# griffithlab/regtools

Hardware: AMD Instinct MI355X
Metric: alignments/sec + junctions/sec, junctions extract, 1/2/4/8 MI355X (higher is better)
Workload: dtype u8/u32 integer; 1 GPU; configs[1]: synthetic 50000000-read 101 bp BAM per GPU, ~15% reads with one N-op, junctions extract -s XS; reads_per_gpu=50000000, seed=1, bgzf_members=169426, compressed_bytes_per_gpu=533101619, inflated_bytes_per_gpu=11060000978

## Files before the change

regtools_amd/csrc/kernels.hip:

```cpp
#include "kernels.h"

#include <mutex>
#include <type_traits>

#include "bam_core.h"
#include "inflate_core.h"
#include "inflate_coop.h"
#include "inflate_ring.h"
#include "inflate_wave.h"

namespace rgx {

__device__ __forceinline__ uint32_t lane_id() { return threadIdx.x & 63u; }
__device__ __forceinline__ uint64_t lanemask_lt() { return (1ull << lane_id()) - 1ull; }

__device__ __forceinline__ uint32_t wave_incl_scan(uint32_t v) {
#pragma unroll
    for (int d = 1; d < 64; d <<= 1) {
        uint32_t t = __shfl_up(v, d, 64);
        if ((int)lane_id() >= d) v += t;
    }
    return v;
}

// ... 686 lines not shown
            if (o < w1) r[j] = ld128(arena + o);
        }
#pragma unroll
        for (int j = 0; j < kChunks; ++j) {
            const uint64_t o = w0 + (uint64_t)j * 1024 + (uint64_t)lane * 16;
            if (o < w1) *(u32x4 *)(s_buf + (o - w0)) = r[j];
        }
    }
    __syncthreads();
    const uint32_t *s_w = (const uint32_t *)s_buf;
    auto lds32 = [&](uint32_t off) -> uint32_t {
        if constexpr (STAGED) return __builtin_amdgcn_alignbyte(s_w[(off >> 2) + 1], s_w[off >> 2], off & 3u);
        else return ld32(arena + w0 + off);
    };
    if (lane * 8 < cnt) {
        uint64_t o = a + seg_cp[(size_t)s * kSegCpSlots + lane];
        const uint32_t k_end = min(cnt, lane * 8 + 8);
        for (uint32_t k = lane * 8; k < k_end; ++k) {
            const uint32_t ro = (uint32_t)(o - w0);
            s_off[k] = ro;
            o += 4 + (uint64_t)((STAGED && o + 4 <= w1) ? lds32(ro) : ld32(arena + o));
        }
    }
    __syncthreads();
    const uint32_t base = seg_base[s];
    DecodeTally t;
    for (uint32_t k = lane; k < cnt; k += 64) {
        const uint32_t ro = s_off[k];
        const uint64_t o = w0 + ro;
        RecHead h;
        {
            const uint32_t sh = ro & 3u, wi = ro >> 2;
            uint32_t x[8];
            if constexpr (STAGED) {
                uint32_t d[9];
#pragma unroll
                for (int q = 0; q < 9; ++q) d[q] = s_w[wi + q];
#pragma unroll
                for (int q = 0; q < 8; ++q) x[q] = __builtin_amdgcn_alignbyte(d[q + 1], d[q], sh);
            } else {
                (void)sh; (void)wi;
#pragma unroll
                for (int q = 0; q < 8; ++q) x[q] = ld32(arena + o + 4 * q);
            }
            rec_head_words(x, h);
        }
        const uint64_t rec_end = o + 4 + (uint64_t)(uint32_t)h.block_len;
        const bool in_win = STAGED && rec_end <= w1;
        const uint32_t cig_ro = ro + 36 + h.l_qname;
        const uint8_t *g_data = arena + o + 36;
        auto cigar_at = [&](uint32_t q) -> uint32_t { return in_win ? lds32(cig_ro + 4 * q) : ld32(g_data + h.l_qname + 4 * (size_t)q); };
        auto tag_strand = [&](uint8_t t0, uint8_t t1, bool *unknown) -> char {
            const int64_t l_data = (int64_t)h.block_len - 32;
            if (in_win) { const uint8_t *body = s_buf + ro + 36; return strand_from_tag(body + h.aux_off, body + l_data, t0, t1, unknown); }
            return strand_from_tag(g_data + h.aux_off, g_data + l_data, t0, t1, unknown);
        };
        decode_record(h, base + k, o, cfg, soa, t, cigar_at, tag_strand);
    }
    const uint32_t n_iter = wave_incl_scan(t.n_iter), n_long = wave_incl_scan(t.n_long);
    if (lane == 63) { seg_iter[s] = n_iter; seg_long[s] = n_long; }
    if (cfg.stop_out) stop_reduce(cfg.stop_out, t.first_stop, t.last_in);
}

__global__ __launch_bounds__(64) void k_decode_sparse(const uint8_t *__restrict__ arena, uint32_t n_seg, const uint64_t *__restrict__ seg_start,
                                                      const uint32_t *__restrict__ seg_base, const uint32_t *__restrict__ seg_cnt, ExtractCfg cfg, ReadSoA soa,
                                                      uint32_t *seg_iter, uint32_t *seg_long, uint32_t s_begin) {
    const uint32_t s = s_begin + blockIdx.x * 64 + threadIdx.x;
    DecodeTally t;
    if (s < n_seg) {
        const uint32_t cnt = seg_cnt[s];
        uint64_t o = cnt ? seg_start[s] : 0;
        const uint32_t base = cnt ? seg_base[s] : 0;
        for (uint32_t k = 0; k < cnt; ++k) {
            RecHead h;
            rec_head(arena + o, h);
            const uint8_t *g_data = arena + o + 36;
            auto cigar_at = [&](uint32_t q) -> uint32_t { return ld32(g_data + h.l_qname + 4 * (size_t)q); };
            auto tag_strand = [&](uint8_t t0, uint8_t t1, bool *unknown) -> char {
                return strand_from_tag(g_data + h.aux_off, g_data + ((int64_t)h.block_len - 32), t0, t1, unknown);
            };
            decode_record(h, base + k, o, cfg, soa, t, cigar_at, tag_strand);
            o += 4 + (uint64_t)(uint32_t)h.block_len;
        }
        seg_iter[s] = t.n_iter; seg_long[s] = t.n_long;
    }
    if (cfg.stop_out) stop_reduce(cfg.stop_out, t.first_stop, t.last_in);
}

__global__ __launch_bounds__(64) void k_long_fill(uint32_t n_seg, const uint32_t *__restrict__ seg_base, const uint32_t *__restrict__ seg_cnt,
                                                  const uint32_t *__restrict__ seg_long_base, ExtractCfg cfg, ReadSoA soa, uint32_t *long_list) {
    const uint32_t s = blockIdx.x, lane = threadIdx.x;
    const uint32_t cnt = seg_cnt[s], base = seg_base[s];
    uint32_t out = seg_long_base[s];
    for (uint32_t k0 = 0; k0 < cnt; k0 += 64) {
        const uint32_t k = k0 + lane;
        bool is_long = false;
        if (k < cnt) is_long = soa.n_ev[base + k] != 0 && (soa.flag_nc[base + k] & 0xffff) > cfg.long_threshold;
        const uint64_t m = __ballot(is_long);
        if (is_long) long_list[out + (uint32_t)__popcll(m & lanemask_lt())] = base + k;
        out += (uint32_t)__popcll(m);
    }
}

const DecodeKnobs &decode_knobs() {
    static const DecodeKnobs k = [] {
        DecodeKnobs v;
        if (const char *e = getenv("REGTOOLS_AMD_DECODE")) {
            v.wave_form = !strncmp(e, "wave", 4);
            if (const char *c = strchr(e, ',')) v.seg_bytes = atoi(c + 1);
        }
        return v;
    }();
    return k;
}
void launch_decode_seg(const uint8_t *arena, SegGeom g, uint32_t n_seg, const uint64_t *seg_start, const uint32_t *seg_base,
                       const uint32_t *seg_cnt, ExtractCfg cfg, ReadSoA soa, uint32_t *seg_iter, uint32_t *seg_long, const uint16_t *seg_cp, bool staged, hipStream_t stream,
                       uint32_t s_begin) {
    if (n_seg <= s_begin) return;
    const uint32_t n = n_seg - s_begin;
    if (staged && g.seg_bytes == kSegBytes) hipLaunchKernelGGL(k_decode_seg<true>, dim3(n), dim3(64), kSegBytes + kSegTail + 48, stream, arena, g, n_seg, seg_start, seg_base, seg_cnt, cfg, soa, seg_iter, seg_long, seg_cp, s_begin);
    else {
        static const bool wave_form = decode_knobs().wave_form;
        if (wave_form && g.seg_bytes == kSegBytes) hipLaunchKernelGGL(k_decode_seg<false>, dim3(n), dim3(64), 0, stream, arena, g, n_seg, seg_start, seg_base, seg_cnt, cfg, soa, seg_iter, seg_long, seg_cp, s_begin);
        else hipLaunchKernelGGL(k_decode_sparse, dim3((n + 63) / 64), dim3(64), 0, stream, arena, n_seg, seg_start, seg_base, seg_cnt, cfg, soa, seg_iter, seg_long, s_begin);
    }
}
__global__ void k_collect_odd_aux(const uint8_t *__restrict__ arena, ReadSoA soa, uint32_t n_rec, uint32_t cap, uint32_t *count, int32_t *out) {
    const uint32_t i = blockIdx.x * blockDim.x + threadIdx.x;
    if (i >= n_rec || !(soa.strand[i] & 0x80u)) return;
    const uint32_t fnc = soa.flag_nc[i];
    const int32_t pos = soa.pos[i];
    const uint32_t k = atomicAdd(count, 1u);
    if (k < cap) { out[3 * (size_t)k] = soa.tid[i]; out[3 * (size_t)k + 1] = pos; out[3 * (size_t)k + 2] = rec_endpos(arena + soa.cig_off[i], fnc & 0xffffu, fnc >> 16, pos); }
}
void launch_collect_odd_aux(const uint8_t *arena, ReadSoA soa, uint32_t n_rec, uint32_t cap, uint32_t *count, int32_t *out, hipStream_t stream) {
    if (n_rec) hipLaunchKernelGGL(k_collect_odd_aux, dim3((n_rec + 255) / 256), dim3(256), 0, stream, arena, soa, n_rec, cap, count, out);
}
void launch_long_fill(uint32_t n_seg, const uint32_t *seg_base, const uint32_t *seg_cnt, const uint32_t *seg_long_base, ExtractCfg cfg, ReadSoA soa,
                      uint32_t *long_list, hipStream_t stream) {
    if (n_seg) hipLaunchKernelGGL(k_long_fill, dim3(n_seg), dim3(64), 0, stream, n_seg, seg_base, seg_cnt, seg_long_base, cfg, soa, long_list);
}


__device__ __forceinline__ void put_event(const EventSoA &ev, uint32_t slot, int32_t tid, uint32_t start, uint32_t end, uint32_t ts,
                                          uint32_t te, char strand, uint32_t rpos, uint32_t rend, uint32_t read) {
    if (ev.read) ev.read[slot] = read;
    ev.tid[slot] = (uint32_t)tid; ev.start[slot] = start;
    ev.ilen_cls[slot] = (end - start) << 2 | strand_class(strand);
    ev.ts[slot] = ts; ev.te[slot] = te; ev.strand[slot] = (uint8_t)strand;
    if (ev.rpos) { ev.rpos[slot] = rpos; ev.rend[slot] = rend; }
}

__global__ void k_emit_short(const uint8_t *__restrict__ arena, uint32_t n_rec, ExtractCfg cfg, ReadSoA soa,
                             const uint32_t *__restrict__ ev_base, EventSoA ev, uint32_t row_begin, const uint32_t *__restrict__ part_totals, uint32_t n_parts, uint32_t slot_cap) {
    uint32_t i = row_begin + blockIdx.x * blockDim.x + threadIdx.x;
    if (i >= n_rec) return;
    uint32_t nev = soa.n_ev[i];
    if (!nev) return;
    uint32_t fnc = soa.flag_nc[i], n_cigar = fnc & 0xffff;
    if (n_cigar > cfg.long_threshold) return;
    const uint8_t *cig = arena + soa.cig_off[i];
    int32_t tid = soa.tid[i];
    char strand = (char)soa.strand[i];
    uint32_t slot = ev_base[i];
    for (uint32_t k = 0; k < n_parts; ++k) slot += part_totals[k];
    const int32_t pos = soa.pos[i];
    const uint32_t rend = ev.rpos ? (uint32_t)rec_endpos(cig, n_cigar, fnc >> 16, pos) : 0u;
    char carried = 0;
    cigar_walk(pos, cig, n_cigar, [&](uint32_t s, uint32_t e, uint32_t ts, uint32_t te) {
        char st = strand;
        if (cfg.fa_data) {
            const FaContig fc = cfg.fa_tab[tid];
            if (!fc.present) { cfg.fa_missing[0] = 1u + (uint32_t)tid; }
            else { const char m = strand_from_motif(cfg.fa_data, fc, s, e, carried); if (m != '?') st = m; }
            carried = st;
        }
        if (intron_ok(s, e, cfg.min_intron, cfg.max_intron)) { if (slot < slot_cap) put_event(ev, slot, tid, s, e, ts, te, st, (uint32_t)pos, rend, i); ++slot; }
    });
}

__global__ __launch_bounds__(256) void k_emit_long(const uint8_t *__restrict__ arena, const uint32_t *__restrict__ long_list,
                                                   uint32_t n_long, ExtractCfg cfg, ReadSoA soa,
                                                   const uint32_t *__restrict__ ev_base, EventSoA ev) {
    __shared__ uint32_t s_ops[4][64];
    __shared__ uint32_t s_R[4][65];
    const uint32_t wave = threadIdx.x >> 6, lane = lane_id();
    const uint32_t stride = gridDim.x * 4;
    uint32_t w = blockIdx.x * 4 + wave;
    if (w >= n_long) return;
    uint32_t nx_i = long_list[w];
    uint32_t nn_i = w + stride < n_long ? long_list[w + stride] : 0u;
    uint32_t nx_fnc = soa.flag_nc[nx_i], nx_slot = ev_base[nx_i];
    uint64_t nx_cig = soa.cig_off[nx_i];
    int32_t nx_tid = soa.tid[nx_i], nx_pos = soa.pos[nx_i];
    uint8_t nx_strand = soa.strand[nx_i];
    for (; w < n_long; w += stride) {
        const uint32_t i = nx_i, fnc = nx_fnc;
        const uint32_t n_cigar = fnc & 0xffff;
        const uint8_t *cig = arena + nx_cig;
        const int32_t tid = nx_tid;
        const char strand = (char)nx_strand;
        uint32_t slot = nx_slot;
        const uint32_t rpos = (uint32_t)nx_pos;
        const uint32_t c_first = lane < n_cigar ? ld32(cig + 4 * (size_t)lane) : 0x5u ;
        if (w + stride < n_long) {
            nx_i = nn_i;
            nx_fnc = soa.flag_nc[nx_i]; nx_slot = ev_base[nx_i]; nx_cig = soa.cig_off[nx_i]; nx_tid = soa.tid[nx_i]; nx_pos = soa.pos[nx_i]; nx_strand = soa.strand[nx_i];
            if (w + 2 * stride < n_long) nn_i = long_list[w + 2 * stride];
        }
        uint32_t rend = 0;
        if (ev.rpos) {
            uint32_t span = 0;
            for (uint32_t t0 = lane; t0 < n_cigar; t0 += 64) span += cig_ref_len(ld32(cig + 4 * (size_t)t0));
            span = __shfl(wave_incl_scan(span), 63, 64);
            rend = ((fnc >> 16) & 4u) ? rpos + 1 : rpos + span;
        }
        uint32_t refpos = rpos;
        uint32_t ts_carry = refpos;
        bool pend = false; uint32_t p_start = 0, p_end = 0, p_ts = 0; char p_strand = strand;
        char carried = 0;
        for (uint32_t t0 = 0; t0 < n_cigar; t0 += 64) {
            const uint32_t k = t0 + lane;
            const uint32_t c = t0 == 0 ? c_first : k < n_cigar ? ld32(cig + 4 * (size_t)k) : 0x5u ;
            s_ops[wave][lane] = c;
            const uint32_t adv = cig_advances_junction_state(c) ? (c >> 4) : 0u;
            const uint32_t incl = wave_incl_scan(adv);
            const uint32_t R_before = refpos + incl - adv, R_after = refpos + incl;
            s_R[wave][lane] = R_before;
            if (lane == 63) s_R[wave][64] = R_after;
            const bool brk = k < n_cigar && cig_is_breaker(c);
            const bool isN = k < n_cigar && cig_is_N(c);
            const uint64_t B = __ballot(brk);
            __builtin_amdgcn_wave_barrier();
            if (pend && B) {
                const uint32_t nb = (uint32_t)__ffsll((unsigned long long)B) - 1;
                const uint32_t te = s_R[wave][nb];
                if (lane == 0 && intron_ok(p_start, p_end, cfg.min_intron, cfg.max_intron)) put_event(ev, slot, tid, p_start, p_end, p_ts, te, p_strand, rpos, rend, i);
                if (intron_ok(p_start, p_end, cfg.min_intron, cfg.max_intron)) ++slot;
                pend = false;
            }
            const uint64_t below = B & lanemask_lt();
            const uint64_t above = lane == 63 ? 0ull : (B >> (lane + 1)) << (lane + 1);
            const uint32_t ts = below ? s_R[wave][(63 - (uint32_t)__clzll((long long)below)) + 1] : ts_carry;
            const bool closed = above != 0;
            const uint32_t te = closed ? s_R[wave][(uint32_t)__ffsll((unsigned long long)above) - 1] : 0u;
            const bool ok = isN && intron_ok(R_before, R_after, cfg.min_intron, cfg.max_intron);
            char my_strand = strand;
            if (cfg.fa_data) {
                const FaContig fc = cfg.fa_tab[tid];
                char sA = strand, sB = strand;
                if (isN) {
                    if (!fc.present) cfg.fa_missing[0] = 1u + (uint32_t)tid;
                    else {
                        const char mA = strand_from_motif(cfg.fa_data, fc, R_before, R_after, 0), mB = strand_from_motif(cfg.fa_data, fc, R_before, R_after, '-');
                        if (mA != '?') sA = mA;
                        if (mB != '?') sB = mB;
                    }
                }
                uint64_t nm = __ballot(isN);
                while (nm) {
                    const uint32_t l = (uint32_t)__ffsll((unsigned long long)nm) - 1; nm &= nm - 1;
                    const char a = (char)__shfl((int)sA, l, 64), b = (char)__shfl((int)sB, l, 64);
                    const char s = carried == '-' ? b : a;
                    if (lane == l) my_strand = s;
                    carried = s;
                }
            }
            const uint64_t emit_mask = __ballot(ok && closed);
            if (ok && closed) put_event(ev, slot + (uint32_t)__popcll(emit_mask & lanemask_lt()), tid, R_before, R_after, ts, te, my_strand, rpos, rend, i);
            slot += (uint32_t)__popcll(emit_mask);
            if (B) {
                const uint32_t lastb = 63 - (uint32_t)__clzll((long long)B);
                const uint32_t lc = s_ops[wave][lastb];
                ts_carry = s_R[wave][lastb + 1];
                if (cig_is_N(lc)) {
                    pend = true;
                    p_start = s_R[wave][lastb]; p_end = s_R[wave][lastb + 1];
                    const uint64_t bl = B & ((1ull << lastb) - 1ull);
                    p_ts = __shfl(ts, lastb, 64);
                    p_strand = (char)__shfl((int)my_strand, lastb, 64);
                    (void)bl;
                }
            }
            refpos = __shfl(R_after, 63, 64);
            __builtin_amdgcn_wave_barrier();
        }
        if (pend && lane == 0 && intron_ok(p_start, p_end, cfg.min_intron, cfg.max_intron)) put_event(ev, slot, tid, p_start, p_end, p_ts, refpos, p_strand, rpos, rend, i);
    }
}

void launch_emit_short(const uint8_t *arena, uint32_t n_rec, ExtractCfg cfg, ReadSoA soa, const uint32_t *ev_base, EventSoA ev,
                       hipStream_t stream, uint32_t row_begin, const uint32_t *part_totals, uint32_t n_parts, uint32_t slot_cap) {
    if (n_rec <= row_begin) return;
    hipLaunchKernelGGL(k_emit_short, dim3((n_rec - row_begin + 255) / 256), dim3(256), 0, stream, arena, n_rec, cfg, soa, ev_base, ev, row_begin, part_totals, n_parts, slot_cap);
}
void launch_emit_long(const uint8_t *arena, const uint32_t *long_list, uint32_t n_long, ExtractCfg cfg,
                      ReadSoA soa, const uint32_t *ev_base, EventSoA ev, hipStream_t stream) {
    if (!n_long) return;
    uint32_t blocks = (n_long + 3) / 4;
    if (blocks > 256 * 8) blocks = 256 * 8;
    hipLaunchKernelGGL(k_emit_long, dim3(blocks), dim3(256), 0, stream, arena, long_list, n_long, cfg, soa, ev_base, ev);
}

constexpr uint32_t kScanTile = 4096;

__device__ __forceinline__ uint32_t block_excl_scan_256(uint32_t v, uint32_t *s_wave , uint32_t &block_total) {
    const uint32_t incl = wave_incl_scan(v);
    const uint32_t w = threadIdx.x >> 6;
    if (lane_id() == 63) s_wave[w] = incl;
    __syncthreads();
    uint32_t off = 0;
#pragma unroll
    for (uint32_t k = 0; k < 4; ++k) off += (k < w) ? s_wave[k] : 0u;
    block_total = s_wave[0] + s_wave[1] + s_wave[2] + s_wave[3];
    __syncthreads();
    return off + incl - v;
}

__global__ __launch_bounds__(256) void k_scan_reduce(const uint32_t *__restrict__ in, uint32_t n, uint32_t *tile_sum) {
    __shared__ uint32_t s_wave[4];
    const uint32_t base = blockIdx.x * kScanTile + threadIdx.x * 16;
    uint32_t sum = 0;
#pragma unroll
    for (uint32_t k = 0; k < 16; ++k) sum += (base + k < n) ? in[base + k] : 0u;
    uint32_t tot; block_excl_scan_256(sum, s_wave, tot);
    if (threadIdx.x == 0) tile_sum[blockIdx.x] = tot;
}

__global__ __launch_bounds__(256) void k_scan_tiles(uint32_t *tile_sum, uint32_t n_tiles, uint32_t *total) {
    __shared__ uint32_t s_wave[4];
    uint32_t carry = 0;
    for (uint32_t base = 0; base < n_tiles; base += 256) {
        const uint32_t i = base + threadIdx.x;
        const uint32_t v = i < n_tiles ? tile_sum[i] : 0u;
        uint32_t tot; const uint32_t ex = block_excl_scan_256(v, s_wave, tot);
        if (i < n_tiles) tile_sum[i] = carry + ex;
        carry += tot;
    }
    if (threadIdx.x == 0 && total) *total = carry;
}

__global__ __launch_bounds__(256) void k_scan_apply(const uint32_t *__restrict__ in, uint32_t *out, uint32_t n, const uint32_t *__restrict__ tile_sum) {
    __shared__ uint32_t s_wave[4];
    const uint32_t base = blockIdx.x * kScanTile + threadIdx.x * 16;
    uint32_t v[16], sum = 0;
#pragma unroll
    for (uint32_t k = 0; k < 16; ++k) { v[k] = (base + k < n) ? in[base + k] : 0u; sum += v[k]; }
    uint32_t tot; uint32_t run = block_excl_scan_256(sum, s_wave, tot) + tile_sum[blockIdx.x];
#pragma unroll
    for (uint32_t k = 0; k < 16; ++k) { if (base + k < n) out[base + k] = run; run += v[k]; }
}

size_t scan_tmp_words(uint32_t n) { return (size_t)(n + kScanTile - 1) / kScanTile + 1; }

void launch_scan_u32(const uint32_t *in, uint32_t *out, uint32_t n, uint32_t *total, uint32_t *tmp, hipStream_t stream) {
    if (!n) { if (total) (void)hipMemsetAsync(total, 0, 4, stream); return; }
    const uint32_t tiles = (n + kScanTile - 1) / kScanTile;
    hipLaunchKernelGGL(k_scan_reduce, dim3(tiles), dim3(256), 0, stream, in, n, tmp);
    hipLaunchKernelGGL(k_scan_tiles, dim3(1), dim3(256), 0, stream, tmp, tiles, total);
    hipLaunchKernelGGL(k_scan_apply, dim3(tiles), dim3(256), 0, stream, in, out, n, tmp);
}

constexpr uint32_t kRadixRowsLarge = 32, kRadixRowsSmall = 8, kRadixSmallMax = 2u << 20;
static inline uint32_t radix_rows(uint32_t n) {
    return n <= kRadixSmallMax ? kRadixRowsSmall : kRadixRowsLarge;
}

__device__ __forceinline__ uint32_t radix_digit(const uint32_t *__restrict__ word, const uint32_t *__restrict__ perm_in, uint32_t i,
                                                uint32_t shift, uint32_t mask, uint32_t &src) {
    src = perm_in ? perm_in[i] : i;
    return (word[src] >> shift) & mask;
}

__device__ __forceinline__ uint64_t match_digit(uint32_t d, bool valid) {
    uint64_t m = __ballot(valid);
#pragma unroll
    for (uint32_t b = 0; b < 8; ++b) {
        const uint64_t bal = __ballot((d >> b) & 1u);
        m &= ((d >> b) & 1u) ? bal : ~bal;
    }
    return m;
}

template <bool KEYED>
__global__ __launch_bounds__(64) void k_radix_hist(const uint32_t *__restrict__ word, uint32_t shift, uint32_t mask,
                                                   const uint32_t *__restrict__ perm_in, uint32_t n, uint32_t n_tiles, uint32_t *hist, uint32_t rows) {
    __shared__ uint32_t s_cnt[256];
    for (uint32_t k = threadIdx.x; k < 256; k += 64) s_cnt[k] = 0;
    __syncthreads();
    const uint32_t base = blockIdx.x * 64 * rows;
    for (uint32_t r = 0; r < rows; ++r) {
        const uint32_t i = base + r * 64 + threadIdx.x;
        if (i < n) { uint32_t src; atomicAdd(&s_cnt[KEYED ? ((word[i] >> shift) & mask) : radix_digit(word, perm_in, i, shift, mask, src)], 1u); }
    }
    __syncthreads();
    for (uint32_t k = threadIdx.x; k < 256; k += 64) hist[(size_t)k * n_tiles + blockIdx.x] = s_cnt[k];
}

template <bool KEYED>
__global__ __launch_bounds__(64) void k_radix_scatter(const uint32_t *__restrict__ word, uint32_t shift, uint32_t mask,
                                                      const uint32_t *__restrict__ perm_in, uint32_t *perm_out, uint32_t n,
                                                      uint32_t n_tiles, const uint32_t *__restrict__ hist_scan, uint32_t *key_out,
                                                      const uint32_t *__restrict__ digit_total, uint32_t rows) {
    __shared__ uint32_t s_base[256];
    {
        const uint32_t k0 = threadIdx.x * 4;
        const uint32_t t0 = digit_total[k0], t1 = digit_total[k0 + 1], t2 = digit_total[k0 + 2], t3 = digit_total[k0 + 3];
        const uint32_t incl = wave_incl_scan(t0 + t1 + t2 + t3);
        uint32_t run = incl - (t0 + t1 + t2 + t3);
        s_base[k0] = run + hist_scan[(size_t)k0 * n_tiles + blockIdx.x]; run += t0;
        s_base[k0 + 1] = run + hist_scan[(size_t)(k0 + 1) * n_tiles + blockIdx.x]; run += t1;
        s_base[k0 + 2] = run + hist_scan[(size_t)(k0 + 2) * n_tiles + blockIdx.x]; run += t2;
        s_base[k0 + 3] = run + hist_scan[(size_t)(k0 + 3) * n_tiles + blockIdx.x];
    }
    __syncthreads();
    const uint32_t base = blockIdx.x * 64 * rows;
    for (uint32_t r = 0; r < rows; ++r) {
        const uint32_t i = base + r * 64 + threadIdx.x;
        const bool valid = i < n;
        uint32_t src = 0, key = 0;
        uint32_t d = 0;
        if (KEYED) { if (valid) { key = word[i]; src = perm_in ? perm_in[i] : i; d = (key >> shift) & mask; } }
        else d = valid ? radix_digit(word, perm_in, i, shift, mask, src) : 0u;
        const uint64_t m = match_digit(d, valid);
        if (valid) {
            const uint32_t rank = (uint32_t)__popcll(m & lanemask_lt());
            const uint32_t leader = (uint32_t)__ffsll((unsigned long long)m) - 1;
            uint32_t b = 0;
            if (lane_id() == leader) { b = s_base[d]; s_base[d] = b + (uint32_t)__popcll(m); }
            b = __shfl(b, leader, 64);
            perm_out[b + rank] = src;
            if (KEYED) key_out[b + rank] = key;
        }
        __builtin_amdgcn_wave_barrier();
    }
}

__global__ __launch_bounds__(256) void k_radix_offsets(uint32_t *hist, uint32_t n_tiles, uint32_t *digit_total) {
    __shared__ uint32_t s_wave[4];
    uint32_t *row = hist + (size_t)blockIdx.x * n_tiles;
    uint32_t carry = 0;
    for (uint32_t base = 0; base < n_tiles; base += 256 * 8) {
        const uint32_t i0 = base + threadIdx.x * 8;
        uint32_t v[8], sum = 0;
#pragma unroll
        for (int k = 0; k < 8; ++k) { v[k] = i0 + k < n_tiles ? row[i0 + k] : 0u; sum += v[k]; }
        uint32_t tot; uint32_t ex = carry + block_excl_scan_256(sum, s_wave, tot);
#pragma unroll
        for (int k = 0; k < 8; ++k) { if (i0 + k < n_tiles) row[i0 + k] = ex; ex += v[k]; }
        carry += tot;
    }
    if (threadIdx.x == 0) digit_total[blockIdx.x] = carry;
}

size_t radix_tmp_words(uint32_t n) {
    const size_t tile = 64 * (size_t)radix_rows(n), tiles = ((size_t)n + tile - 1) / tile;
    const size_t n_small = std::min<size_t>(n, kRadixSmallMax), tile_small = 64 * (size_t)radix_rows((uint32_t)n_small);
    const size_t tiles_small = (n_small + tile_small - 1) / tile_small;
    return 256 * std::max(tiles, tiles_small) + 256 + 4;
}

void launch_radix_pass(const uint32_t *word, uint32_t shift, uint32_t bits, const uint32_t *perm_in, uint32_t *perm_out, uint32_t n,
                       uint32_t *tmp, hipStream_t stream) {
    if (!n) return;
    const uint32_t rows = radix_rows(n), tiles = (n + 64 * rows - 1) / (64 * rows);
    const uint32_t mask = (1u << bits) - 1u;
    uint32_t *hist = tmp, *totals = tmp + (size_t)256 * tiles;
    hipLaunchKernelGGL(k_radix_hist<false>, dim3(tiles), dim3(64), 0, stream, word, shift, mask, perm_in, n, tiles, hist, rows);
    hipLaunchKernelGGL(k_radix_offsets, dim3(256), dim3(256), 0, stream, hist, tiles, totals);
    hipLaunchKernelGGL(k_radix_scatter<false>, dim3(tiles), dim3(64), 0, stream, word, shift, mask, perm_in, perm_out, n, tiles, hist, (uint32_t *)nullptr, totals, rows);
}
void launch_radix_pass_keyed(const uint32_t *key_in, uint32_t *key_out, uint32_t shift, uint32_t bits, const uint32_t *perm_in, uint32_t *perm_out,
                             uint32_t n, uint32_t *tmp, hipStream_t stream) {
    if (!n) return;
    const uint32_t rows = radix_rows(n), tiles = (n + 64 * rows - 1) / (64 * rows);
    const uint32_t mask = (1u << bits) - 1u;
    uint32_t *hist = tmp, *totals = tmp + (size_t)256 * tiles;
    hipLaunchKernelGGL(k_radix_hist<true>, dim3(tiles), dim3(64), 0, stream, key_in, shift, mask, perm_in, n, tiles, hist, rows);
    hipLaunchKernelGGL(k_radix_offsets, dim3(256), dim3(256), 0, stream, hist, tiles, totals);
    hipLaunchKernelGGL(k_radix_scatter<true>, dim3(tiles), dim3(64), 0, stream, key_in, shift, mask, perm_in, perm_out, n, tiles, hist, key_out, totals, rows);
}


__device__ __forceinline__ bool bgzf_magic_at(const uint8_t *__restrict__ p) {
    if (p[0] != 31 || p[1] != 139) return false;
    return p[2] == 8 && (p[3] & 4) && p[10] == 6 && p[11] == 0 && p[12] == 'B' && p[13] == 'C' && p[14] == 2 && p[15] == 0;
}

__device__ __forceinline__ uint32_t magic_mask16(const uint8_t *__restrict__ bam, uint64_t len, uint64_t base) {
    uint32_t m = 0;
    if (base + 16 + 18 <= len) {
        u32x4 a = ld128(bam + base), b = ld128(bam + base + 16);
        uint8_t w[32];
        *(u32x4 *)w = a; *(u32x4 *)(w + 16) = b;
#pragma unroll
        for (int k = 0; k < 16; ++k)
            if (w[k] == 31 && w[k + 1] == 139) { if (bgzf_magic_at(bam + base + k)) m |= 1u << k; }
    } else {
        for (int k = 0; k < 16; ++k) if (base + k + 18 <= len && bgzf_magic_at(bam + base + k)) m |= 1u << k;
    }
    return m;
}

__global__ __launch_bounds__(256) void k_magic_count(const uint8_t *__restrict__ bam, uint64_t len, uint32_t *tile_cnt) {
    __shared__ uint32_t s_wave[4];
    const uint64_t base = (uint64_t)blockIdx.x * kMagicTile + threadIdx.x * 16;
    const uint32_t c = (uint32_t)__popc(magic_mask16(bam, len, base));
    uint32_t tot; block_excl_scan_256(c, s_wave, tot);
    if (threadIdx.x == 0) tile_cnt[blockIdx.x] = tot;
}

__global__ __launch_bounds__(256) void k_magic_fill(const uint8_t *__restrict__ bam, uint64_t len, const uint32_t *__restrict__ tile_base, uint64_t *cand) {
    __shared__ uint32_t s_wave[4];
    const uint64_t base = (uint64_t)blockIdx.x * kMagicTile + threadIdx.x * 16;
    uint32_t m = magic_mask16(bam, len, base);
    uint32_t tot; uint32_t slot = tile_base[blockIdx.x] + block_excl_scan_256((uint32_t)__popc(m), s_wave, tot);
    while (m) { const uint32_t k = (uint32_t)__ffs((int)m) - 1; m &= m - 1; cand[slot++] = base + k; }
}

__global__ void k_member_link(const uint8_t *__restrict__ bam, uint64_t len, const uint64_t *__restrict__ cand, uint32_t n, uint32_t *next,
                              uint32_t *isize, uint32_t *reach, uint64_t root2) {
    const uint32_t i = blockIdx.x * blockDim.x + threadIdx.x;
    if (i >= n) return;
    const uint64_t off = cand[i];
    const uint64_t blen = (uint64_t)ld16(bam + off + 16) + 1;
    uint32_t nx = n, isz = 0xffffffffu;
    if (blen >= 26 && off + blen <= len) {
        isz = ld32(bam + off + blen - 4);
        if (isz == 0xffffffffu) isz = 0xfffffffeu;
        const uint64_t want = off + blen;
        uint32_t lo = i + 1, hi = n;
        while (lo < hi) { const uint32_t mid = (lo + hi) >> 1; if (cand[mid] < want) lo = mid + 1; else hi = mid; }
        if (lo < n && cand[lo] == want) nx = lo;
    } else nx = 0xffffffffu;
    next[i] = nx; isize[i] = isz;
    reach[i] = ((i == 0 && off == 0) || off == root2) ? 1u : 0u;
}

__global__ void k_member_jump(uint32_t n, const uint32_t *__restrict__ next_in, uint32_t *next_out, uint32_t *reach) {
    const uint32_t i = blockIdx.x * blockDim.x + threadIdx.x;
    if (i >= n) return;
    const uint32_t nx = next_in[i];
    if (nx < n) {
        if (reach[i]) reach[nx] = 1u;
        next_out[i] = next_in[nx];
    } else next_out[i] = nx;
}

__global__ void k_member_compact(const uint8_t *__restrict__ bam, uint64_t len, const uint64_t *__restrict__ cand, const uint32_t *__restrict__ isize,
                                 const uint32_t *__restrict__ reach, const uint32_t *__restrict__ rank, uint32_t n, Member *members, uint32_t *isize_compact) {
    const uint32_t i = blockIdx.x * blockDim.x + threadIdx.x;
    if (i >= n || !reach[i]) return;
    const uint64_t off = cand[i];
    const uint32_t blen = (uint32_t)ld16(bam + off + 16) + 1;
    const uint32_t r = rank[i];
    Member m; m.cpos = off + 18; m.upos = 0; m.isize = isize[i];
    m.clen = blen >= 26 ? blen - 18 : 0;
    if (m.cpos + m.clen + 8 > len) m.clen = len > m.cpos + 8 ? (uint32_t)(len - 8 - m.cpos) : 0;
    members[r] = m;
    isize_compact[r] = (isize[i] <= kBgzfMaxBlock) ? isize[i] : 0u;
}

__global__ __launch_bounds__(256) void k_member_upos(Member *members, const uint32_t *__restrict__ isz, const uint32_t *__restrict__ n_ptr, uint64_t *total) {
    __shared__ uint32_t s_wave[4];
    const uint32_t n = *n_ptr;
    uint64_t carry = 0;
    for (uint32_t base = 0; base < n; base += 2048) {
        const uint32_t i0 = base + threadIdx.x * 8;
        uint32_t v[8], sum = 0;
#pragma unroll
        for (int k = 0; k < 8; ++k) { v[k] = i0 + k < n ? isz[i0 + k] : 0u; sum += v[k]; }
        uint32_t tot; uint32_t ex = block_excl_scan_256(sum, s_wave, tot);
#pragma unroll
        for (int k = 0; k < 8; ++k) { if (i0 + k < n) members[i0 + k].upos = carry + ex; ex += v[k]; }
        carry += tot;
    }
    if (threadIdx.x == 0) *total = carry;
}

__global__ void k_member_query(const Member *__restrict__ members, const uint32_t *__restrict__ n_ptr, const uint64_t *__restrict__ q_coff, uint32_t n_q,
                               uint32_t *q_index, uint64_t *q_upos) {
    const uint32_t k = blockIdx.x * blockDim.x + threadIdx.x;
    if (k >= n_q) return;
    const uint32_t n = *n_ptr;
    const uint64_t want = q_coff[k] + 18;
    uint32_t lo = 0, hi = n;
    while (lo < hi) { const uint32_t mid = (lo + hi) >> 1; if (members[mid].cpos < want) lo = mid + 1; else hi = mid; }
    const bool hit = lo < n && members[lo].cpos == want;
    q_index[k] = hit ? lo : n;
    q_upos[k] = hit ? members[lo].upos : ~0ull;
}

__global__ void k_member_fix(Member *members, uint32_t *isize_compact, const uint32_t *__restrict__ n_ptr, const uint32_t *__restrict__ fix) {
    const uint32_t i = blockIdx.x * blockDim.x + threadIdx.x;
    if (i >= *n_ptr) return;
    const uint32_t sz = fix[i];
    members[i].isize = sz;
    isize_compact[i] = sz <= kBgzfMaxBlock ? sz : 0u;
}
__global__ void k_member_stop(const Member *__restrict__ members, const uint32_t *__restrict__ n_ptr, const uint32_t *__restrict__ from_ptr, uint32_t *stop) {
    const uint32_t n = *n_ptr;
    const uint32_t i = blockIdx.x * blockDim.x + threadIdx.x;
    if (i < *from_ptr) return;
    if (i < n && (members[i].isize == 0 || members[i].isize > kBgzfMaxBlock)) atomicMin(stop, i);
}

void launch_magic_count(const uint8_t *bam, uint64_t len, uint32_t n_tiles, uint32_t *tile_cnt, hipStream_t stream) {
    if (n_tiles) hipLaunchKernelGGL(k_magic_count, dim3(n_tiles), dim3(256), 0, stream, bam, len, tile_cnt);
}
void launch_magic_fill(const uint8_t *bam, uint64_t len, uint32_t n_tiles, const uint32_t *tile_base, uint64_t *cand, hipStream_t stream) {
    if (n_tiles) hipLaunchKernelGGL(k_magic_fill, dim3(n_tiles), dim3(256), 0, stream, bam, len, tile_base, cand);
}
void launch_member_link(const uint8_t *bam, uint64_t len, const uint64_t *cand, uint32_t n, uint32_t *next, uint32_t *isize, uint32_t *reach,
                        uint64_t root2, hipStream_t stream) {
    if (n) hipLaunchKernelGGL(k_member_link, dim3((n + 255) / 256), dim3(256), 0, stream, bam, len, cand, n, next, isize, reach, root2);
}
void launch_member_jump(uint32_t n, const uint32_t *next_in, uint32_t *next_out, uint32_t *reach, hipStream_t stream) {
    if (n) hipLaunchKernelGGL(k_member_jump, dim3((n + 255) / 256), dim3(256), 0, stream, n, next_in, next_out, reach);
}
void launch_member_compact(const uint8_t *bam, uint64_t len, const uint64_t *cand, const uint32_t *isize, const uint32_t *reach, const uint32_t *rank, uint32_t n,
                           Member *members, uint32_t *isize_compact, hipStream_t stream) {
    if (n) hipLaunchKernelGGL(k_member_compact, dim3((n + 255) / 256), dim3(256), 0, stream, bam, len, cand, isize, reach, rank, n, members, isize_compact);
}
void launch_member_upos(Member *members, const uint32_t *isize_compact, const uint32_t *n_members, uint64_t *total, hipStream_t stream) {
    hipLaunchKernelGGL(k_member_upos, dim3(1), dim3(256), 0, stream, members, isize_compact, n_members, total);
}
void launch_member_query(const Member *members, const uint32_t *n_members, const uint64_t *q_coff, uint32_t n_q, uint32_t *q_index, uint64_t *q_upos,
                         hipStream_t stream) {
    if (n_q) hipLaunchKernelGGL(k_member_query, dim3((n_q + 63) / 64), dim3(64), 0, stream, members, n_members, q_coff, n_q, q_index, q_upos);
}
void launch_member_fix(Member *members, uint32_t *isize_compact, uint32_t max_members, const uint32_t *n_members, const uint32_t *fix, hipStream_t stream) {
    if (max_members) hipLaunchKernelGGL(k_member_fix, dim3((max_members + 255) / 256), dim3(256), 0, stream, members, isize_compact, n_members, fix);
}
void launch_member_stop(const Member *members, uint32_t max_members, const uint32_t *n_members, const uint32_t *from, uint32_t *stop, hipStream_t stream) {
    if (max_members) hipLaunchKernelGGL(k_member_stop, dim3((max_members + 255) / 256), dim3(256), 0, stream, members, n_members, from, stop);
}

__global__ void k_heads(EventSoA ev, const uint32_t *__restrict__ perm, uint32_t n, uint32_t *head) {
    const uint32_t i = blockIdx.x * blockDim.x + threadIdx.x;
    if (i >= n) return;
    uint32_t h = 1;
    if (i > 0) {
        const uint32_t a = perm[i], b = perm[i - 1];
        h = (ev.tid[a] != ev.tid[b]) || (ev.start[a] != ev.start[b]) || (ev.ilen_cls[a] != ev.ilen_cls[b]);
    }
    head[i] = h;
}

__global__ void k_reduce(EventSoA ev, const uint32_t *__restrict__ perm, const uint32_t *__restrict__ head,
                         const uint32_t *__restrict__ seg_excl, uint32_t n, UniqueSoA u, uint32_t *head_pos) {
    const uint32_t i = blockIdx.x * blockDim.x + threadIdx.x;
    const bool valid = i < n;
    uint32_t row = 0, ts = 0xffffffffu, te = 0, hd = 0;
    if (valid) {
        const uint32_t e = perm[i];
        hd = head[i];
        row = seg_excl[i] + hd - 1;
        ts = ev.ts[e]; te = ev.te[e];
        if (hd) {
            head_pos[row] = i;
            u.tid[row] = ev.tid[e]; u.start[row] = ev.start[e]; u.end[row] = ev.start[e] + (ev.ilen_cls[e] >> 2);
            u.first_seen[row] = e;
// ... 195 lines not shown
```

Baseline: 2.187 billion alignments/s.

## Rewrite u32 prefix scan with DPP wave scans, coalesced rows, single-kernel small path

Reworks the three-pass exclusive scan. Each block now covers 8192 elements loaded as coalesced 64-wide rows instead of per-thread contiguous strides of 16. Wave-level inclusive scans use DPP row shifts and broadcasts instead of shuffle loops. Inputs that fit in one tile run a single-block kernel, skipping the reduce and apply launches. This cuts launch count and memory transactions for scans, at the cost of more registers per thread and non-portable DPP intrinsics.

```diff
diff --git a/regtools_amd/csrc/kernels.hip b/regtools_amd/csrc/kernels.hip
--- a/regtools_amd/csrc/kernels.hip
+++ b/regtools_amd/csrc/kernels.hip
@@ -1012,7 +1012,8 @@
     hipLaunchKernelGGL(k_emit_long, dim3(blocks), dim3(256), 0, stream, arena, long_list, n_long, cfg, soa, ev_base, ev);
 }
 
-constexpr uint32_t kScanTile = 4096;
+constexpr uint32_t kScanRows = 32, kScanTile = 256 * kScanRows;
+constexpr uint32_t kScanTripRows = 4, kScanTrip = 256 * kScanTripRows;
 
 __device__ __forceinline__ uint32_t block_excl_scan_256(uint32_t v, uint32_t *s_wave , uint32_t &block_total) {
     const uint32_t incl = wave_incl_scan(v);
@@ -1027,47 +1028,93 @@
     return off + incl - v;
 }
 
-__global__ __launch_bounds__(256) void k_scan_reduce(const uint32_t *__restrict__ in, uint32_t n, uint32_t *tile_sum) {
+__device__ __forceinline__ uint32_t scan_wave_incl(uint32_t x) {
+    int v = (int)x;
+    v += __builtin_amdgcn_update_dpp(0, v, 0x111, 0xf, 0xf, false);
+    v += __builtin_amdgcn_update_dpp(0, v, 0x112, 0xf, 0xf, false);
+    v += __builtin_amdgcn_update_dpp(0, v, 0x114, 0xf, 0xf, false);
+    v += __builtin_amdgcn_update_dpp(0, v, 0x118, 0xf, 0xf, false);
+    v += __builtin_amdgcn_update_dpp(0, v, 0x142, 0xa, 0xf, false);
+    v += __builtin_amdgcn_update_dpp(0, v, 0x143, 0xc, 0xf, false);
+    return (uint32_t)v;
+}
+
+template <uint32_t kRows, bool kFull>
+__device__ __forceinline__ void scan_load_rows(const uint32_t *in, uint32_t rem, uint32_t (&v)[kRows]) {
+    const uint32_t o = (threadIdx.x >> 6) * (kRows * 64) + lane_id();
+#pragma unroll
+    for (uint32_t j = 0; j < kRows; ++j) v[j] = (kFull || o + j * 64 < rem) ? in[o + j * 64] : 0u;
+}
+
+__device__ __forceinline__ uint32_t scan_wave_offset(uint32_t wave_sum, uint32_t *s_wave , uint32_t &tile_total) {
+    const uint32_t w = threadIdx.x >> 6;
+    if (lane_id() == 0) s_wave[w] = wave_sum;
+    __syncthreads();
+    uint32_t off = 0;
+#pragma unroll
+    for (uint32_t k = 0; k < 4; ++k) off += (k < w) ? s_wave[k] : 0u;
+    tile_total = s_wave[0] + s_wave[1] + s_wave[2] + s_wave[3];
+    __syncthreads();
+    return off;
+}
+
+template <uint32_t kRows, bool kFull>
+__device__ __forceinline__ uint32_t scan_tile(const uint32_t *in, uint32_t *out, uint32_t rem, uint32_t carry, uint32_t *s_wave) {
+    uint32_t v[kRows];
+    scan_load_rows<kRows, kFull>(in, rem, v);
+    uint32_t run = 0;
+#pragma unroll
+    for (uint32_t j = 0; j < kRows; ++j) {
+        const uint32_t incl = scan_wave_incl(v[j]);
+        v[j] = run + incl - v[j];
+        run += (uint32_t)__builtin_amdgcn_readlane((int)incl, 63);
+    }
+    uint32_t tot; carry += scan_wave_offset(run, s_wave, tot);
+    const uint32_t o = (threadIdx.x >> 6) * (kRows * 64) + lane_id();
+#pragma unroll
+    for (uint32_t j = 0; j < kRows; ++j) if (kFull || o + j * 64 < rem) out[o + j * 64] = carry + v[j];
+    return tot;
+}
+
+__global__ __launch_bounds__(256) void k_scan_reduce(const uint32_t *in, uint32_t n, uint32_t *tile_sum) {
     __shared__ uint32_t s_wave[4];
-    const uint32_t base = blockIdx.x * kScanTile + threadIdx.x * 16;
+    const uint32_t base = blockIdx.x * kScanTile, rem = n - base;
+    uint32_t v[kScanRows];
+    if (rem >= kScanTile) scan_load_rows<kScanRows, true>(in + base, rem, v); else scan_load_rows<kScanRows, false>(in + base, rem, v);
     uint32_t sum = 0;
 #pragma unroll
-    for (uint32_t k = 0; k < 16; ++k) sum += (base + k < n) ? in[base + k] : 0u;
-    uint32_t tot; block_excl_scan_256(sum, s_wave, tot);
+    for (uint32_t j = 0; j < kScanRows; ++j) sum += v[j];
+    sum = (uint32_t)__builtin_amdgcn_readlane((int)scan_wave_incl(sum), 63);
+    uint32_t tot; scan_wave_offset(sum, s_wave, tot);
     if (threadIdx.x == 0) tile_sum[blockIdx.x] = tot;
 }
 
-__global__ __launch_bounds__(256) void k_scan_tiles(uint32_t *tile_sum, uint32_t n_tiles, uint32_t *total) {
+__global__ __launch_bounds__(256) void k_scan_tiles(const uint32_t *in, uint32_t *out, uint32_t n, uint32_t *total) {
     __shared__ uint32_t s_wave[4];
     uint32_t carry = 0;
-    for (uint32_t base = 0; base < n_tiles; base += 256) {
-        const uint32_t i = base + threadIdx.x;
-        const uint32_t v = i < n_tiles ? tile_sum[i] : 0u;
-        uint32_t tot; const uint32_t ex = block_excl_scan_256(v, s_wave, tot);
-        if (i < n_tiles) tile_sum[i] = carry + ex;
-        carry += tot;
+    for (uint32_t base = 0;; base += kScanTrip) {
+        const uint32_t rem = n - base;
+        carry += scan_tile<kScanTripRows, false>(in + base, out + base, rem, carry, s_wave);
+        if (rem <= kScanTrip) break;
     }
     if (threadIdx.x == 0 && total) *total = carry;
 }
 
-__global__ __launch_bounds__(256) void k_scan_apply(const uint32_t *__restrict__ in, uint32_t *out, uint32_t n, const uint32_t *__restrict__ tile_sum) {
+__global__ __launch_bounds__(256) void k_scan_apply(const uint32_t *in, uint32_t *out, uint32_t n, const uint32_t *tile_sum) {
     __shared__ uint32_t s_wave[4];
-    const uint32_t base = blockIdx.x * kScanTile + threadIdx.x * 16;
-    uint32_t v[16], sum = 0;
-#pragma unroll
-    for (uint32_t k = 0; k < 16; ++k) { v[k] = (base + k < n) ? in[base + k] : 0u; sum += v[k]; }
-    uint32_t tot; uint32_t run = block_excl_scan_256(sum, s_wave, tot) + tile_sum[blockIdx.x];
-#pragma unroll
-    for (uint32_t k = 0; k < 16; ++k) { if (base + k < n) out[base + k] = run; run += v[k]; }
-}
-
-size_t scan_tmp_words(uint32_t n) { return (size_t)(n + kScanTile - 1) / kScanTile + 1; }
+    const uint32_t base = blockIdx.x * kScanTile, rem = n - base, carry = tile_sum[blockIdx.x];
+    if (rem >= kScanTile) scan_tile<kScanRows, true>(in + base, out + base, rem, carry, s_wave);
+    else scan_tile<kScanRows, false>(in + base, out + base, rem, carry, s_wave);
+}
+
+size_t scan_tmp_words(uint32_t n) { return ((size_t)n + kScanTile - 1) / kScanTile + 1; }
 
 void launch_scan_u32(const uint32_t *in, uint32_t *out, uint32_t n, uint32_t *total, uint32_t *tmp, hipStream_t stream) {
     if (!n) { if (total) (void)hipMemsetAsync(total, 0, 4, stream); return; }
-    const uint32_t tiles = (n + kScanTile - 1) / kScanTile;
+    if (n <= kScanTile) { hipLaunchKernelGGL(k_scan_tiles, dim3(1), dim3(256), 0, stream, in, out, n, total); return; }
+    const uint32_t tiles = (n - 1) / kScanTile + 1;
     hipLaunchKernelGGL(k_scan_reduce, dim3(tiles), dim3(256), 0, stream, in, n, tmp);
-    hipLaunchKernelGGL(k_scan_tiles, dim3(1), dim3(256), 0, stream, tmp, tiles, total);
+    hipLaunchKernelGGL(k_scan_tiles, dim3(1), dim3(256), 0, stream, tmp, tmp, tiles, total);
     hipLaunchKernelGGL(k_scan_apply, dim3(tiles), dim3(256), 0, stream, in, out, n, tmp);
 }
 
```

Measured after the change: 2.205 billion alignments/s, median of 3. Within noise of the previous version (+0.8%).
